# DoHoonKim8/stark-verifier

Hardware: AMD Instinct MI355X
Metric: recursive plonky2 proofs/sec (Semaphore d=20) (higher is better)
Workload: dtype u64 (Goldilocks field, integer); 1 GPU; recursive: per unit one Semaphore signal (group 2^20, n=2^13, blowup 8, 28 FRI queries, 16 PoW bits, zk) + the recursive proof verifying it (n=2^14, same FRI parameters); 128 units per GPU per step, 10 prover contexts per GPU; all_gather of (nullifier|topic) + Poseidon aggregation root per step; parallelism=independent proofs sharded over ranks, no data-path collective, exchange=none (one rank): gl355_aggregation_root over the local leaves, units_proven_in_process=1674

## Files before the change

include/gl355.h:

```cpp
#ifndef GL355_H
#define GL355_H
#include <stddef.h>
#include <stdint.h>

#ifdef __cplusplus
extern "C" {
#endif

#define GL355_OK 0
#define GL355_E_INVALID_ARG (-1)
#define GL355_E_NO_DEVICE (-2)
#define GL355_E_OOM (-3)
#define GL355_E_HIP (-4)
#define GL355_E_UNSUPPORTED (-5)
#define GL355_E_WITNESS (-6)
#define GL355_E_VERIFY (-7)

#define GL355_P UINT64_C(0xFFFFFFFF00000001)
#define GL355_COSET_SHIFT UINT64_C(7)
#define GL355_SALT_SIZE 4
#define GL355_MAX_FRI_ARITY_BITS 4
#define GL355_MAX_UNITS 16

typedef struct gl355_ctx gl355_ctx;
// ... 303 lines not shown
int32_t gl355_bn254_g1_fixed_base_mul(gl355_ctx* ctx, const uint64_t base[8], const uint64_t* scalars , uint64_t n, uint64_t* out );
int32_t gl355_bn254_g1_fft(gl355_ctx* ctx, uint64_t* points , uint32_t log_n, int32_t inverse);
typedef struct gl355_msm_bases gl355_msm_bases;
int32_t gl355_bn254_g1_msm_prepare(gl355_ctx* ctx, const uint64_t* points , uint64_t n, gl355_msm_bases** out);
int32_t gl355_bn254_g1_msm_prepared(gl355_ctx* ctx, const gl355_msm_bases* bases, const uint64_t* scalars , uint32_t n_sets,
                                    uint64_t* results );
int32_t gl355_bn254_g1_msm_bases_free(gl355_ctx* ctx, gl355_msm_bases* bases);

int32_t gl355_kzg_setup(gl355_ctx* ctx, const uint64_t tau[4], uint32_t log_n, uint64_t* g , uint64_t* g_lagrange );
int32_t gl355_kzg_lagrange_from_powers(gl355_ctx* ctx, const uint64_t* g , uint64_t n_points, uint32_t log_n,
                                       uint64_t* g_lagrange );
int32_t gl355_kzg_commit(gl355_ctx* ctx, const uint64_t* g , const uint64_t* poly , uint32_t log_n, int32_t values_form,
                         uint64_t result[8]);
int32_t gl355_kzg_open(gl355_ctx* ctx, const uint64_t* g, const uint64_t* coeffs, uint32_t log_n, const uint64_t z[4], uint64_t eval[4],
                       uint64_t witness[8], uint64_t* quotient );

typedef struct gl355_plonk_pk gl355_plonk_pk;
enum { GL355_PLONK_STAGE_ADVICE = 0, GL355_PLONK_STAGE_LOOKUP_PERMUTE = 1, GL355_PLONK_STAGE_PERMUTATION = 2, GL355_PLONK_STAGE_LOOKUP_PRODUCT = 3,
       GL355_PLONK_STAGE_VANISHING_RANDOM = 4, GL355_PLONK_STAGE_EVALUATE_H = 5, GL355_PLONK_STAGE_QUOTIENT_COMMIT = 6, GL355_PLONK_STAGE_EVALUATIONS = 7,
       GL355_PLONK_STAGE_SHPLONK = 8, GL355_PLONK_STAGES = 9 };
int32_t gl355_keccak256(const uint8_t* data, uint64_t len, uint8_t out[32]);
int32_t gl355_kzg_commit_columns(gl355_ctx* ctx, const uint64_t* g, const uint64_t* columns, uint32_t log_n, uint32_t n_cols, uint64_t* results );
int32_t gl355_plonk_keygen(gl355_ctx* ctx, const uint64_t* desc, uint64_t desc_words, const uint64_t* g, const uint64_t* g_lagrange, const uint64_t* fixed_values,
                           const uint32_t* mapping, gl355_plonk_pk** out);
int32_t gl355_plonk_pk_info(const gl355_plonk_pk* pk, uint64_t info[8]);
int32_t gl355_plonk_pk_commitments(const gl355_plonk_pk* pk, uint64_t* fixed_commitments, uint64_t* sigma_commitments);
int32_t gl355_plonk_pk_digest(const gl355_plonk_pk* pk, uint64_t digest[4]);
int32_t gl355_plonk_pk_set_digest(gl355_plonk_pk* pk, const uint64_t digest[4]);
int32_t gl355_plonk_pk_export_quotient(gl355_plonk_pk* pk, uint64_t* host_out );
int32_t gl355_plonk_prove(gl355_ctx* ctx, gl355_plonk_pk* pk, const uint64_t* advice, const uint64_t* instances, const uint32_t* instance_lens, const uint8_t seed[32],
                          uint8_t* proof, uint64_t capacity, uint64_t* proof_len, uint64_t* trace, double* stage_ms);
int32_t gl355_plonk_pk_destroy(gl355_plonk_pk* pk);

enum { GL355_PLONK_FAIL_GATE = 0, GL355_PLONK_FAIL_GATE_POISONED = 1, GL355_PLONK_FAIL_LOOKUP = 2, GL355_PLONK_FAIL_PERMUTATION = 3 };
int32_t gl355_plonk_check_witness(gl355_ctx* ctx, const uint64_t* desc, uint64_t desc_words, const uint64_t* fixed_values, const uint32_t* mapping ,
                                  const uint64_t* advice, const uint64_t* instances, const uint32_t* instance_lens, uint32_t* failures ,
                                  uint64_t capacity, uint64_t* n_failures, double* stage_ms );

typedef struct gl355_halo2_tape gl355_halo2_tape;
int32_t gl355_halo2_tape_load(gl355_ctx* ctx, const uint64_t* tape, uint64_t n_words, uint64_t n_inputs, uint32_t k, uint32_t n_advice, gl355_halo2_tape** out);
int32_t gl355_halo2_tape_free(gl355_halo2_tape* tape);
int32_t gl355_halo2_synthesize(gl355_ctx* ctx, const gl355_halo2_tape* tape, const uint64_t* inputs, uint64_t* advice_out, uint64_t* status );
int32_t gl355_halo2_tape_launches(const gl355_halo2_tape* tape, uint64_t* out );
int32_t gl355_halo2_synthesize_host(const uint64_t* tape, uint64_t n_words, uint64_t n_inputs, uint32_t k, uint32_t n_advice, const uint64_t* inputs,
                                    uint64_t* advice_out, uint64_t* status );

typedef struct gl355_plonk_vk gl355_plonk_vk;
int32_t gl355_bn254_g2_mul(const uint64_t scalar[4], const uint64_t* point , uint64_t out[16]);
int32_t gl355_bn254_pairing_check(const uint64_t* g1 , const uint64_t* g2 , uint32_t n, int32_t* ok);
int32_t gl355_plonk_vk_create(const uint64_t* desc, uint64_t desc_words, const uint64_t* fixed_commitments, const uint64_t* sigma_commitments,
                              const uint64_t digest[4] , const uint64_t s_g2[16], gl355_plonk_vk** out);
int32_t gl355_plonk_vk_from_pk(const gl355_plonk_pk* pk, const uint64_t s_g2[16], gl355_plonk_vk** out);
int32_t gl355_plonk_vk_destroy(gl355_plonk_vk* vk);
int32_t gl355_plonk_verify(gl355_ctx* ctx , const gl355_plonk_vk* vk, const uint64_t* instances, const uint32_t* instance_lens,
                           const uint8_t* proof, uint64_t proof_len, int32_t* ok);
int32_t gl355_plonk_verify_batch(gl355_ctx* ctx , const gl355_plonk_vk* vk, uint32_t n_proofs, const uint64_t* instances ,
                                 const uint32_t* instance_lens , const uint8_t* const* proofs, const uint64_t* proof_lens,
                                 const uint8_t seed[32], int32_t* ok, int32_t* first_bad );
const char* gl355_plonk_verify_last_error(void);
int32_t gl355_plonk_verify_stage_ms(double ms[3]);
int32_t gl355_kzg_params_check(gl355_ctx* ctx, const uint64_t* g , uint64_t n_points, const uint64_t* g_lagrange ,
                               uint32_t log_n, const uint64_t s_g2[16], const uint8_t seed[32], int32_t* ok);

int32_t gl355_zs_partial_products(gl355_ctx* ctx, const uint64_t* wires, const uint64_t* sigmas,
                                  const uint64_t* k_is, uint32_t log_n, uint32_t n_routed,
                                  uint32_t max_degree, uint64_t beta, uint64_t gamma,
                                  uint64_t* z_out, uint64_t* pp_out);

enum { GL355_BN_M_MUL = 0, GL355_BN_M_ADD = 1, GL355_BN_M_SUB = 2, GL355_BN_M_CANON = 3, GL355_BN_M_FROM_INT = 4, GL355_BN_M_TO_INT = 5,
       GL355_BN_M_INV = 6, GL355_BN_M_IS_ZERO = 7, GL355_BN_M_EQ = 8, GL355_BN_FQ = 16,
       GL355_BN_F29_MUL = 32, GL355_BN_F29_MUL_FR = 33, GL355_BN_F29_ADD_NORM = 34, GL355_BN_F29_SUB_C2 = 35, GL355_BN_F29_SUB_C4 = 36,
       GL355_BN_F29_SUB_C8 = 37, GL355_BN_F29_SUB_C16 = 38, GL355_BN_F29_NEG_C2 = 39, GL355_BN_F29_FROM_U256 = 40, GL355_BN_F29_TO_U256 = 41,
       GL355_BN_F29_LIFT = 42, GL355_BN_F29_LIFT_INL = 43, GL355_BN_F29_LOWER = 44, GL355_BN_F29_IS_ZERO_MOD = 45, GL355_BN_F29_TABLE_FORM = 46,
       GL355_BN_F29_NORM = 47, GL355_BN_HASH_FR_ENTER = 48, GL355_BN_HASH_FR_LEAVE = 49 };
enum { GL355_BN_CHAIN_XYZZ = 0, GL355_BN_CHAIN_JAC29 = 1, GL355_BN_CHAIN_JAC = 2, GL355_BN_CHAIN_RED29_LIFT = 3, GL355_BN_CHAIN_RED29_RAW = 4,
       GL355_BN_CHAIN_J = 5 };
enum { GL355_BN_STEP_ADD = 0, GL355_BN_STEP_DOUBLE = 1, GL355_BN_STEP_ACC = 2, GL355_BN_STEP_SELF = 3, GL355_BN_STEP_MADD = 4 };
int32_t gl355_bn254_arith_batch(gl355_ctx* ctx, int32_t op, const uint32_t* a , const uint32_t* b , uint32_t* out ,
                                uint64_t n);
int32_t gl355_bn254_g1_chain(gl355_ctx* ctx, int32_t form, const uint32_t* operands , uint32_t n_operands,
                             const uint32_t* steps , uint32_t n_chains, uint32_t n_steps, uint32_t* trace );

enum { GL355_GL_MUL = 0, GL355_GL_MUL_MULTI1 = 1, GL355_GL_MUL_MULTI2 = 2, GL355_GL_MUL_MULTI3 = 3, GL355_GL_MUL_MULTI4 = 4, GL355_GL_MUL_FILL = 5,
       GL355_GL_MUL2_FILL = 6, GL355_GL_SQR = 7, GL355_GL_SBOX = 8, GL355_GL_SBOX4 = 9, GL355_GL_RECOMBINE = 10, GL355_GL_RECOMBINE_MULTI4 = 11 };
int32_t gl355_gl_arith_batch(gl355_ctx* ctx, int32_t op, const uint64_t* a , const uint64_t* b , uint64_t* out , uint64_t n);
int32_t gl355_poseidon_permute_lanes(gl355_ctx* ctx, int32_t form, uint64_t* states , uint64_t count);


int32_t gl355_bn254_g1_msm_bits(gl355_ctx* ctx, const uint64_t* points, const gl355_msm_bases* bases , const uint64_t* scalars, uint64_t n,
                                uint32_t n_sets, uint32_t max_bits, uint64_t* results , uint32_t plan_out[4] );
int32_t gl355_plonk_pk_commit_columns(gl355_plonk_pk* pk, uint32_t which, const uint64_t* columns , uint32_t sets, uint64_t tail,
                                      uint64_t* results );

#ifdef __cplusplus
}
#endif
#endif
```

stark-verifier_amd/csrc/gl_hook.hip:

```cpp
#include "gl355_internal.h"
#include "poseidon_lanes.cuh"

namespace gl355 {

static int hk_gl_width(int32_t op) {
    switch (op) {
    case GL355_GL_MUL: case GL355_GL_MUL_MULTI1: case GL355_GL_MUL_FILL: case GL355_GL_SQR: case GL355_GL_SBOX: case GL355_GL_RECOMBINE: return 1;
    case GL355_GL_MUL_MULTI2: case GL355_GL_MUL2_FILL: return 2;
    case GL355_GL_MUL_MULTI3: return 3;
    case GL355_GL_MUL_MULTI4: case GL355_GL_SBOX4: case GL355_GL_RECOMBINE_MULTI4: return 4;
    default: return 0;
    }
}

template <int N> GL_DEV void hk_mul_multi(const uint64_t* a, const uint64_t* b, uint64_t* out) {
    uint64_t x[N], y[N], r[N];
#pragma unroll
    for (int j = 0; j < N; j++) { x[j] = a[j]; y[j] = b[j]; }
    gl_mul_multi<N>(x, y, r);
#pragma unroll
    for (int j = 0; j < N; j++) out[j] = r[j];
}

struct HkRow {
    uint64_t xr[5], al, ah;
    GL_DEV HkRow(uint64_t a, uint64_t b) {
#pragma unroll
        for (int k = 0; k < 5; k++) xr[k] = a * (uint64_t)(k + 1) + b;
        al = (uint32_t)b; ah = b >> 32;
    }
    GL_DEV void term(int k) {
        al += (uint64_t)(uint32_t)xr[k] * PSD_CIRC_DEV[k];
        ah += (uint64_t)(uint32_t)(xr[k] >> 32) * PSD_CIRC_DEV[k];
    }
};

__global__ void __launch_bounds__(256) gl_arith_hook_kernel(int32_t op, int32_t width, const uint64_t* a, const uint64_t* b, uint64_t* out, uint64_t n) {
    const uint64_t i = (blockIdx.x * (uint64_t)blockDim.x + threadIdx.x) * (uint64_t)width;
    if (i >= n) return;
    const uint64_t* pa = a + i;
    const uint64_t* pb = b + i;
    uint64_t* po = out + i;
    switch (op) {
    case GL355_GL_MUL: po[0] = gl_mul(pa[0], pb[0]); break;
    case GL355_GL_MUL_MULTI1: hk_mul_multi<1>(pa, pb, po); break;
    case GL355_GL_MUL_MULTI2: hk_mul_multi<2>(pa, pb, po); break;
    case GL355_GL_MUL_MULTI3: hk_mul_multi<3>(pa, pb, po); break;
    case GL355_GL_MUL_MULTI4: hk_mul_multi<4>(pa, pb, po); break;
    case GL355_GL_MUL_FILL: {
        HkRow row(pa[0], pb[0]);
        po[0] = gl_mul_fill(pa[0], pb[0], [&](int k) { row.term(k); });
        po[n] = row.al; po[2 * n] = row.ah;
        break;
    }
    case GL355_GL_MUL2_FILL: {
        HkRow row(pa[0], pb[0]);
        const uint64_t x[2] = {pa[0], pa[1]}, y[2] = {pb[0], pb[1]};
        uint64_t r[2];
        gl_mul2_fill(x, y, r, [&](int k) { row.term(k); });
        po[0] = r[0]; po[1] = r[1];
        po[n] = row.al; po[2 * n] = row.ah;
        po[n + 1] = 0; po[2 * n + 1] = 0;
        break;
    }
    case GL355_GL_SQR: po[0] = gl_sqr(pa[0]); break;
    case GL355_GL_SBOX: po[0] = psd_sbox(pa[0]); break;
    case GL355_GL_SBOX4: {
        uint64_t x0 = pa[0], x1 = pa[1], x2 = pa[2], x3 = pa[3];
        psd_sbox4(x0, x1, x2, x3);
        po[0] = x0; po[1] = x1; po[2] = x2; po[3] = x3;
        break;
    }
    case GL355_GL_RECOMBINE: po[0] = psd_recombine(pa[0], pb[0]); break;
    default: {
        const uint64_t al[4] = {pa[0], pa[1], pa[2], pa[3]}, ah[4] = {pb[0], pb[1], pb[2], pb[3]};
        uint64_t r[4];
        psd_recombine_multi<4>(al, ah, r);
        po[0] = r[0]; po[1] = r[1]; po[2] = r[2]; po[3] = r[3];
        break;
    }
    }
}

template <int FORM>
__global__ void __launch_bounds__(64) poseidon_lanes_hook_kernel(uint64_t* states, uint64_t count) {
    __shared__ uint64_t rings[4][24];
    const int li = threadIdx.x & 15, grp = threadIdx.x >> 4;
    uint64_t g = blockIdx.x * 4ull + grp;
    const bool valid = g < count;
    if (!valid) g = 0;
    uint64_t s = (li < 12) ? states[g * 12 + li] : 0;
    s = psd_permute_lanes<FORM>(s, li, rings[grp]);
    if (valid && li < 12) states[g * 12 + li] = gl_canon(s);
}

}

using namespace gl355;

extern "C" {
int32_t gl355_gl_arith_batch(gl355_ctx* h, int32_t op, const uint64_t* a, const uint64_t* b, uint64_t* out, uint64_t n) {
    Ctx* ctx = ctx_of(h);
    if (!ctx) return GL355_E_INVALID_ARG;
    if (hipSetDevice(ctx->device) != hipSuccess) return ctx->fail(GL355_E_HIP, "hipSetDevice failed");
    const int width = hk_gl_width(op);
    if (!width) return ctx->fail(GL355_E_INVALID_ARG, "gl_arith_batch: bad op");
    if (n % (uint64_t)width) return ctx->fail(GL355_E_INVALID_ARG, "gl_arith_batch: n is not a multiple of the op's records per lane");
    if (n == 0) return GL355_OK;
    const bool two = !(op == GL355_GL_SQR || op == GL355_GL_SBOX || op == GL355_GL_SBOX4);
    if (!a || !out || (two && !b)) return ctx->fail(GL355_E_INVALID_ARG, "gl_arith_batch: null argument");
    const uint64_t lanes = n / (uint64_t)width;
    if ((lanes + 255) / 256 > 0x7FFFFFFFull) return ctx->fail(GL355_E_UNSUPPORTED, "gl_arith_batch: too many records");
    const uint64_t out_words = (op == GL355_GL_MUL_FILL || op == GL355_GL_MUL2_FILL) ? 3 * n : n;
    Staged sa(ctx), sb(ctx), so(ctx);
    GL355_TRY(sa.open(a, n * 8, 1));
    GL355_TRY(sb.open(two ? b : a, n * 8, 1));
    GL355_TRY(so.open(out, out_words * 8, 2));
    hipLaunchKernelGGL(gl_arith_hook_kernel, dim3((uint32_t)((lanes + 255) / 256)), dim3(256), 0, ctx->stream, op, (int32_t)width, sa.as<const uint64_t>(),
                       sb.as<const uint64_t>(), so.as<uint64_t>(), n);
    GL355_HIP(ctx, hipGetLastError());
    return so.finish();
}

int32_t gl355_poseidon_permute_lanes(gl355_ctx* h, int32_t form, uint64_t* states, uint64_t count) {
    Ctx* ctx = ctx_of(h);
    if (!ctx) return GL355_E_INVALID_ARG;
    if (hipSetDevice(ctx->device) != hipSuccess) return ctx->fail(GL355_E_HIP, "hipSetDevice failed");
    if (form != 0 && form != 3) return ctx->fail(GL355_E_INVALID_ARG, "poseidon_permute_lanes: form is 0 or 3");
    if (count == 0) return GL355_OK;
    if (!states) return ctx->fail(GL355_E_INVALID_ARG, "poseidon_permute_lanes: null states");
    if ((count + 3) / 4 > 0x7FFFFFFFull) return ctx->fail(GL355_E_UNSUPPORTED, "poseidon_permute_lanes: too many states");
    Staged s(ctx);
    GL355_TRY(s.open(states, count * 96, 3));
    const dim3 grid((uint32_t)((count + 3) / 4)), block(64);
    if (form == 3) hipLaunchKernelGGL(poseidon_lanes_hook_kernel<3>, grid, block, 0, ctx->stream, s.as<uint64_t>(), count);
    else hipLaunchKernelGGL(poseidon_lanes_hook_kernel<0>, grid, block, 0, ctx->stream, s.as<uint64_t>(), count);
    GL355_HIP(ctx, hipGetLastError());
    return s.finish();
}
}
```

stark-verifier_amd/csrc/poseidon.cuh:

```cuda
#pragma once
#include "gl_field.cuh"
#if GL_MUL_VARIANT != 1
#error "poseidon.cuh is written on the inline-asm product and its lock-step groups: GL_MUL_VARIANT 1"
#endif

#define PSD_TABLE_QUAL __device__ __constant__ const
#include "poseidon_tables.h"

namespace gl355 {

GL_DEV uint64_t psd_sbox(uint64_t x) {
    const uint64_t x2 = gl_sqr(x);
    const uint64_t a[2] = {x, x2}, b[2] = {x2, x2};
    uint64_t r[2];
    gl_mul_multi<2>(a, b, r);
    return gl_mul(r[0], r[1]);
}

GL_DEV uint64_t psd_recombine(uint64_t al, uint64_t ah) {
    uint32_t t1 = (uint32_t)(al >> 32), top;
    asm("v_add_co_u32_e32 %0, vcc, %0, %2\n\t" GL_HAZARD_NOP "v_addc_co_u32_e32 %1, vcc, 0, %3, vcc"
        : "+v"(t1), "=v"(top) : "v"((uint32_t)ah), "v"((uint32_t)(ah >> 32)) : "vcc");
    return gl_dev_add_mul_eps(((uint64_t)t1 << 32) | (uint32_t)al, top);
}

GL_DEV void psd_sbox4(uint64_t& x0, uint64_t& x1, uint64_t& x2, uint64_t& x3) {
    const uint64_t a[4] = {x0, x1, x2, x3};
    uint64_t sq[4], c3[4], c4[4], o[4];
    gl_mul_multi<4>(a, a, sq);
    gl_mul_multi<4>(a, sq, c3);
    gl_mul_multi<4>(sq, sq, c4);
    gl_mul_multi<4>(c3, c4, o);
    x0 = o[0]; x1 = o[1]; x2 = o[2]; x3 = o[3];
}
template <int N>
GL_DEV void psd_recombine_multi(const uint64_t (&al)[N], const uint64_t (&ah)[N], uint64_t (&out)[N]) {
    static_assert(N >= 3, "three or more: no wait states of their own");
    uint32_t t1[N], top[N], m[N];
    uint64_t c[N], r[N];
#pragma unroll
    for (int j = 0; j < N; j++) {
        asm("v_add_co_u32_e64 %0, %1, %2, %3" : "=v"(t1[j]), "=s"(c[j]) : "v"((uint32_t)(al[j] >> 32)), "v"((uint32_t)ah[j]));
        __builtin_amdgcn_sched_barrier(0);
    }
#pragma unroll
    for (int j = 0; j < N; j++) {
        asm("v_addc_co_u32_e64 %0, %1, 0, %2, %1" : "=v"(top[j]), "+s"(c[j]) : "v"((uint32_t)(ah[j] >> 32)));
        __builtin_amdgcn_sched_barrier(0);
    }
#pragma unroll
    for (int j = 0; j < N; j++) {
        const uint64_t x = ((uint64_t)t1[j] << 32) | (uint32_t)al[j];
        asm("v_mad_u64_u32 %0, %1, %2, -1, %3" : "=v"(r[j]), "=s"(c[j]) : "v"(top[j]), "v"(x));
        __builtin_amdgcn_sched_barrier(0);
    }
#pragma unroll
    for (int j = 0; j < N; j++) {
        asm("v_cndmask_b32_e64 %0, 0, -1, %1" : "=v"(m[j]) : "s"(c[j]));
        __builtin_amdgcn_sched_barrier(0);
    }
#pragma unroll
    for (int j = 0; j < N; j++) out[j] = r[j] + (uint64_t)m[j];
}

#define PSD_MDS_CHAIN(C0)                                                                                  \
    "v_mad_u64_u32 %0, %1, %2, " #C0 ", %14\n\tv_mad_u64_u32 %0, %1, %3, 15, %0\n\tv_mad_u64_u32 %0, %1, %4, 41, %0\n\t" \
    "v_mad_u64_u32 %0, %1, %5, 16, %0\n\tv_mad_u64_u32 %0, %1, %6, 2, %0\n\tv_mad_u64_u32 %0, %1, %7, 28, %0\n\t"      \
    "v_mad_u64_u32 %0, %1, %8, 13, %0\n\tv_mad_u64_u32 %0, %1, %9, 13, %0\n\tv_mad_u64_u32 %0, %1, %10, 39, %0\n\t"    \
    "v_mad_u64_u32 %0, %1, %11, 18, %0\n\tv_mad_u64_u32 %0, %1, %12, 34, %0\n\tv_mad_u64_u32 %0, %1, %13, 20, %0"
template <int R>
GL_DEV uint64_t psd_mds_chain(const uint32_t (&x)[12], uint64_t addend) {
    uint64_t acc, unused;
#define PSD_X(i) "v"(x[((i) + R) % 12])
    if constexpr (R == 0)
        asm(PSD_MDS_CHAIN(25) : "=&v"(acc), "=&s"(unused) : PSD_X(0), PSD_X(1), PSD_X(2), PSD_X(3), PSD_X(4), PSD_X(5), PSD_X(6),
            PSD_X(7), PSD_X(8), PSD_X(9), PSD_X(10), PSD_X(11), "s"(addend));
    else
        asm(PSD_MDS_CHAIN(17) : "=&v"(acc), "=&s"(unused) : PSD_X(0), PSD_X(1), PSD_X(2), PSD_X(3), PSD_X(4), PSD_X(5), PSD_X(6),
            PSD_X(7), PSD_X(8), PSD_X(9), PSD_X(10), PSD_X(11), "s"(addend));
#undef PSD_X
    return acc;
}
template <int R>
GL_DEV void psd_mds_rows(uint64_t (&s)[12], const uint32_t (&lo)[12], const uint32_t (&hi)[12], const uint64_t* rc) {
    if constexpr (R < 12) {
        const uint64_t c0 = rc[R], c1 = rc[R + 1], c2 = rc[R + 2], c3 = rc[R + 3];
        const uint64_t al[4] = {psd_mds_chain<R>(lo, (uint32_t)c0), psd_mds_chain<R + 1>(lo, (uint32_t)c1), psd_mds_chain<R + 2>(lo, (uint32_t)c2),
                                psd_mds_chain<R + 3>(lo, (uint32_t)c3)};
        const uint64_t ah[4] = {psd_mds_chain<R>(hi, c0 >> 32), psd_mds_chain<R + 1>(hi, c1 >> 32), psd_mds_chain<R + 2>(hi, c2 >> 32),
                                psd_mds_chain<R + 3>(hi, c3 >> 32)};
        uint64_t o[4];
        __builtin_amdgcn_sched_barrier(0);
        psd_recombine_multi<4>(al, ah, o);
        s[R] = o[0]; s[R + 1] = o[1]; s[R + 2] = o[2]; s[R + 3] = o[3];
        psd_mds_rows<R + 4>(s, lo, hi, rc);
    }
}
GL_DEV void psd_mds(uint64_t (&s)[12], const uint64_t* rc) {
    uint32_t lo[12], hi[12];
#pragma unroll
    for (int i = 0; i < 12; i++) { lo[i] = (uint32_t)s[i]; hi[i] = (uint32_t)(s[i] >> 32); }
    psd_mds_rows<0>(s, lo, hi, rc);
}


#undef PSD_TABLE_QUAL
#define PSD_TABLE_QUAL __device__ __constant__
#include "poseidon_ktables.h"

GL_DEV void psd_split(uint64_t x, uint32_t (&l)[3]) {
    const uint32_t lo = (uint32_t)x, hi = (uint32_t)(x >> 32);
    l[0] = lo & 0x3FFFFFu;
    l[1] = __builtin_amdgcn_alignbit(hi, lo, 22) & 0x3FFFFFu;
    l[2] = hi >> 12;
}
typedef const __attribute__((address_space(4))) uint64_t* psd_ktab;
GL_DEV void psd_mac(uint64_t& lo, uint64_t& hi, const uint32_t (&l)[3], const uint64_t (&c)[3]) {
    const uint64_t c0 = c[0], c1 = c[1], c2 = c[2];
    uint64_t unused;
    asm("v_mad_u64_u32 %0, %2, %3, %9, %0\n\tv_mad_u64_u32 %1, %2, %4, %9, %1\n\t"
        "v_mad_u64_u32 %0, %2, %5, %10, %0\n\tv_mad_u64_u32 %1, %2, %6, %10, %1\n\t"
        "v_mad_u64_u32 %0, %2, %7, %11, %0\n\tv_mad_u64_u32 %1, %2, %8, %11, %1"
        : "+v"(lo), "+v"(hi), "=&s"(unused)
        : "s"((uint32_t)c0), "s"((uint32_t)(c0 >> 32)), "s"((uint32_t)c1), "s"((uint32_t)(c1 >> 32)), "s"((uint32_t)c2), "s"((uint32_t)(c2 >> 32)),
          "v"(l[0]), "v"(l[1]), "v"(l[2]));
}
GL_DEV void psd_mac_first(uint64_t& lo, uint64_t& hi, const uint32_t (&l)[3], const uint64_t (&c)[3], const uint64_t (&add)[2]) {
    const uint64_t c0 = c[0], c1 = c[1], c2 = c[2];
    uint64_t unused;
    asm("v_mov_b64 %0, %12\n\tv_mov_b64 %1, %13\n\t"
        "v_mad_u64_u32 %0, %2, %3, %9, %0\n\tv_mad_u64_u32 %1, %2, %4, %9, %1\n\t"
        "v_mad_u64_u32 %0, %2, %5, %10, %0\n\tv_mad_u64_u32 %1, %2, %6, %10, %1\n\t"
        "v_mad_u64_u32 %0, %2, %7, %11, %0\n\tv_mad_u64_u32 %1, %2, %8, %11, %1"
        : "=&v"(lo), "=&v"(hi), "=&s"(unused)
        : "s"((uint32_t)c0), "s"((uint32_t)(c0 >> 32)), "s"((uint32_t)c1), "s"((uint32_t)(c1 >> 32)), "s"((uint32_t)c2), "s"((uint32_t)(c2 >> 32)),
          "v"(l[0]), "v"(l[1]), "v"(l[2]), "s"(add[0]), "s"(add[1]));
}
constexpr int psd_k_group = 5;
struct PsdK {
    uint64_t w[psd_k_group][3];
    uint64_t a[2];
};
template <int N, bool WITH_ADD>
GL_DEV void psd_kload(PsdK& k, psd_ktab c, psd_ktab add) {
#pragma unroll
    for (int i = 0; i < N; i++)
#pragma unroll
        for (int j = 0; j < 3; j++) k.w[i][j] = c[3 * i + j];
    if constexpr (WITH_ADD) { k.a[0] = add[0]; k.a[1] = add[1]; }
}
template <int NX, bool HAS_NEXT, int XCAP>
GL_DEV void psd_dot(const uint32_t (&ul)[11][3], const uint32_t (&xl)[XCAP][3], psd_ktab c, PsdK& k, psd_ktab add_next, uint64_t& lo, uint64_t& hi) {
    constexpr int G = psd_k_group, NT = 11 + NX, NG = (NT + G - 1) / G;
    PsdK cur = k;
#pragma unroll
    for (int g = 0; g < NG; g++) {
        const int n = NT - g * G < G ? NT - g * G : G;
        PsdK nxt;
#pragma unroll
        for (int i = 0; i < G; i++) {
            const int t = g * G + i;
            if (t == 0) psd_mac_first(lo, hi, ul[0], cur.w[0], cur.a);
            else if (i < n) {
                if (t < 11) psd_mac(lo, hi, ul[t], cur.w[i]);
                else psd_mac(lo, hi, xl[t - 11], cur.w[i]);
            }
            if (i == 0) {
                __builtin_amdgcn_sched_barrier(0);
                if (g + 1 < NG) {
                    if (NT - (g + 1) * G >= G) psd_kload<G, false>(nxt, c + 3 * (g + 1) * G, add_next);
                    else psd_kload<(NT % G ? NT % G : G), false>(nxt, c + 3 * (g + 1) * G, add_next);
                } else if constexpr (HAS_NEXT) {
                    psd_kload<G, true>(nxt, c + 3 * NT, add_next);
                }
                __builtin_amdgcn_sched_barrier(0);
            }
        }
        __builtin_amdgcn_sched_barrier(0);
        if (g + 1 < NG || HAS_NEXT) cur = nxt;
    }
    if constexpr (HAS_NEXT) k = cur;
}
template <int J>
GL_DEV void psd_block_lane0(const uint32_t (&ul)[11][3], uint32_t (&xl)[PSD_K_BLOCK][3], psd_ktab mac, psd_ktab add, PsdK& k) {
    if constexpr (J < PSD_K_BLOCK) {
        uint64_t lo, hi;
        psd_dot<J, true>(ul, xl, mac + 3 * (11 * (J - 1) + (J - 1) * J / 2), k, add + 2 * J, lo, hi);
        psd_split(psd_sbox(psd_recombine(lo, hi)), xl[J]);
        __builtin_amdgcn_sched_barrier(0);
        psd_block_lane0<J + 1>(ul, xl, mac, add, k);
    }
}
template <int R>
GL_DEV void psd_block_out(uint64_t (&s)[12], const uint32_t (&ul)[11][3], const uint32_t (&xl)[PSD_K_BLOCK][3], psd_ktab mac, psd_ktab add, PsdK& k) {
    constexpr int B = PSD_K_BLOCK;
    if constexpr (R < 12) {
        uint64_t lo, hi;
        psd_dot<B, (R < 11)>(ul, xl, mac + 3 * (11 * (B - 1) + (B - 1) * B / 2 + (11 + B) * R), k, add + 2 * (B + R), lo, hi);
        s[R] = psd_recombine(lo, hi);
        __builtin_amdgcn_sched_barrier(0);
        psd_block_out<R + 1>(s, ul, xl, mac, add, k);
    }
}
GL_DEV void psd_partial_rounds_block(uint64_t (&s)[12]) {
    constexpr int B = PSD_K_BLOCK;
#pragma unroll 1
    for (int blk = 0; blk < 22 / B; blk++) {
        psd_ktab add = (psd_ktab)PSD_K_ADD + blk * 2 * (B - 1 + 12);
        psd_ktab mac = (psd_ktab)PSD_K_MAC;
        asm volatile("" : "+s"(mac));
        PsdK k;
        psd_kload<psd_k_group, true>(k, mac, add);
        __builtin_amdgcn_sched_barrier(0);
        uint32_t ul[11][3], xl[B][3];
#pragma unroll
        for (int i = 0; i < 11; i++) psd_split(s[i + 1], ul[i]);
        psd_split(psd_sbox(s[0]), xl[0]);
        __builtin_amdgcn_sched_barrier(0);
        psd_block_lane0<1>(ul, xl, mac, add, k);
        psd_block_out<0>(s, ul, xl, mac, add, k);
    }
}

constexpr int psd_rounds_per_iter = 2;
GL_DEV void psd_dense_rounds(uint64_t (&s)[12], int r0, int r1) {
#pragma unroll 1
    for (int r = r0; r < r1; r += psd_rounds_per_iter) {
#pragma unroll
        for (int h = 0; h < psd_rounds_per_iter; h++) {
#pragma unroll
            for (int i = 0; i < 12; i += 4) psd_sbox4(s[i], s[i + 1], s[i + 2], s[i + 3]);
            psd_mds(s, &PSD_ALL_RC[12 * (r + h + 1)]);
        }
    }
}
GL_DEV void psd_permute(uint64_t (&s)[12]) {
#pragma unroll
    for (int i = 0; i < 12; i++) s[i] = gl_add_canonical(s[i], PSD_ALL_RC[i]);
    psd_dense_rounds(s, 0, 4);
    psd_partial_rounds_block(s);
    psd_dense_rounds(s, 26, 30);
}

struct PsdSponge {
    uint64_t s[12];
    GL_DEV void init() {
#pragma unroll
        for (int i = 0; i < 12; i++) s[i] = 0;
    }
};

}
```

Baseline: 332.1 recursive proofs/s.

## Restructure Poseidon partial rounds into 3-round blocks with small MDS-derived constants

Replaces the old partial-round block scheme, which split state limbs into 22-bit pieces and used 64-bit constants, with a new 3-round block form. Each output is now a dot product of full 32-bit halves times small (22-bit or narrower) constants, using two mad_u64_u32 per term. This runs 7 blocks of 3 rounds (21) plus one final sbox and MDS round, with new precomputed tables. It also adds a test hook op for the partial rounds. The intent is to cut multiply count and scalar-constant loads in the Poseidon hot path. The risk lies in accumulator overflow bounds and the correctness of the new tables.

```diff
diff --git a/include/gl355.h b/include/gl355.h
--- a/include/gl355.h
+++ b/include/gl355.h
@@ -409,7 +409,8 @@
                              const uint32_t* steps , uint32_t n_chains, uint32_t n_steps, uint32_t* trace );
 
 enum { GL355_GL_MUL = 0, GL355_GL_MUL_MULTI1 = 1, GL355_GL_MUL_MULTI2 = 2, GL355_GL_MUL_MULTI3 = 3, GL355_GL_MUL_MULTI4 = 4, GL355_GL_MUL_FILL = 5,
-       GL355_GL_MUL2_FILL = 6, GL355_GL_SQR = 7, GL355_GL_SBOX = 8, GL355_GL_SBOX4 = 9, GL355_GL_RECOMBINE = 10, GL355_GL_RECOMBINE_MULTI4 = 11 };
+       GL355_GL_MUL2_FILL = 6, GL355_GL_SQR = 7, GL355_GL_SBOX = 8, GL355_GL_SBOX4 = 9, GL355_GL_RECOMBINE = 10, GL355_GL_RECOMBINE_MULTI4 = 11,
+       GL355_GL_PARTIAL_ROUNDS = 13 };
 int32_t gl355_gl_arith_batch(gl355_ctx* ctx, int32_t op, const uint64_t* a , const uint64_t* b , uint64_t* out , uint64_t n);
 int32_t gl355_poseidon_permute_lanes(gl355_ctx* ctx, int32_t form, uint64_t* states , uint64_t count);
 
diff --git a/stark-verifier_amd/csrc/gl_hook.hip b/stark-verifier_amd/csrc/gl_hook.hip
--- a/stark-verifier_amd/csrc/gl_hook.hip
+++ b/stark-verifier_amd/csrc/gl_hook.hip
@@ -9,6 +9,7 @@
     case GL355_GL_MUL_MULTI2: case GL355_GL_MUL2_FILL: return 2;
     case GL355_GL_MUL_MULTI3: return 3;
     case GL355_GL_MUL_MULTI4: case GL355_GL_SBOX4: case GL355_GL_RECOMBINE_MULTI4: return 4;
+    case GL355_GL_PARTIAL_ROUNDS: return 12;
     default: return 0;
     }
 }
@@ -72,6 +73,15 @@
         break;
     }
     case GL355_GL_RECOMBINE: po[0] = psd_recombine(pa[0], pb[0]); break;
+    case GL355_GL_PARTIAL_ROUNDS: {
+        uint64_t s[12];
+#pragma unroll
+        for (int j = 0; j < 12; j++) s[j] = pa[j];
+        psd_partial_rounds_b3(s);
+#pragma unroll
+        for (int j = 0; j < 12; j++) po[j] = s[j];
+        break;
+    }
     default: {
         const uint64_t al[4] = {pa[0], pa[1], pa[2], pa[3]}, ah[4] = {pb[0], pb[1], pb[2], pb[3]};
         uint64_t r[4];
@@ -107,7 +117,7 @@
     if (!width) return ctx->fail(GL355_E_INVALID_ARG, "gl_arith_batch: bad op");
     if (n % (uint64_t)width) return ctx->fail(GL355_E_INVALID_ARG, "gl_arith_batch: n is not a multiple of the op's records per lane");
     if (n == 0) return GL355_OK;
-    const bool two = !(op == GL355_GL_SQR || op == GL355_GL_SBOX || op == GL355_GL_SBOX4);
+    const bool two = !(op == GL355_GL_SQR || op == GL355_GL_SBOX || op == GL355_GL_SBOX4 || op == GL355_GL_PARTIAL_ROUNDS);
     if (!a || !out || (two && !b)) return ctx->fail(GL355_E_INVALID_ARG, "gl_arith_batch: null argument");
     const uint64_t lanes = n / (uint64_t)width;
     if ((lanes + 255) / 256 > 0x7FFFFFFFull) return ctx->fail(GL355_E_UNSUPPORTED, "gl_arith_batch: too many records");
diff --git a/stark-verifier_amd/csrc/poseidon.cuh b/stark-verifier_amd/csrc/poseidon.cuh
--- a/stark-verifier_amd/csrc/poseidon.cuh
+++ b/stark-verifier_amd/csrc/poseidon.cuh
@@ -81,8 +81,8 @@
 #undef PSD_X
     return acc;
 }
-template <int R>
-GL_DEV void psd_mds_rows(uint64_t (&s)[12], const uint32_t (&lo)[12], const uint32_t (&hi)[12], const uint64_t* rc) {
+template <int R, class RC>
+GL_DEV void psd_mds_rows(uint64_t (&s)[12], const uint32_t (&lo)[12], const uint32_t (&hi)[12], RC rc) {
     if constexpr (R < 12) {
         const uint64_t c0 = rc[R], c1 = rc[R + 1], c2 = rc[R + 2], c3 = rc[R + 3];
         const uint64_t al[4] = {psd_mds_chain<R>(lo, (uint32_t)c0), psd_mds_chain<R + 1>(lo, (uint32_t)c1), psd_mds_chain<R + 2>(lo, (uint32_t)c2),
@@ -93,133 +93,112 @@
         __builtin_amdgcn_sched_barrier(0);
         psd_recombine_multi<4>(al, ah, o);
         s[R] = o[0]; s[R + 1] = o[1]; s[R + 2] = o[2]; s[R + 3] = o[3];
-        psd_mds_rows<R + 4>(s, lo, hi, rc);
-    }
-}
-GL_DEV void psd_mds(uint64_t (&s)[12], const uint64_t* rc) {
+        psd_mds_rows<R + 4, RC>(s, lo, hi, rc);
+    }
+}
+template <class RC>
+GL_DEV void psd_mds(uint64_t (&s)[12], RC rc) {
     uint32_t lo[12], hi[12];
 #pragma unroll
     for (int i = 0; i < 12; i++) { lo[i] = (uint32_t)s[i]; hi[i] = (uint32_t)(s[i] >> 32); }
-    psd_mds_rows<0>(s, lo, hi, rc);
+    psd_mds_rows<0, RC>(s, lo, hi, rc);
 }
 
 
 #undef PSD_TABLE_QUAL
 #define PSD_TABLE_QUAL __device__ __constant__
-#include "poseidon_ktables.h"
-
-GL_DEV void psd_split(uint64_t x, uint32_t (&l)[3]) {
-    const uint32_t lo = (uint32_t)x, hi = (uint32_t)(x >> 32);
-    l[0] = lo & 0x3FFFFFu;
-    l[1] = __builtin_amdgcn_alignbit(hi, lo, 22) & 0x3FFFFFu;
-    l[2] = hi >> 12;
-}
-typedef const __attribute__((address_space(4))) uint64_t* psd_ktab;
-GL_DEV void psd_mac(uint64_t& lo, uint64_t& hi, const uint32_t (&l)[3], const uint64_t (&c)[3]) {
-    const uint64_t c0 = c[0], c1 = c[1], c2 = c[2];
+#include "poseidon_b3tables.h"
+
+typedef const __attribute__((address_space(4))) uint32_t* psd_b3tab;
+typedef const __attribute__((address_space(4))) uint64_t* psd_b3add;
+GL_DEV void psd_b3_term(uint64_t& lo, uint64_t& hi, uint32_t c, uint64_t v) {
     uint64_t unused;
-    asm("v_mad_u64_u32 %0, %2, %3, %9, %0\n\tv_mad_u64_u32 %1, %2, %4, %9, %1\n\t"
-        "v_mad_u64_u32 %0, %2, %5, %10, %0\n\tv_mad_u64_u32 %1, %2, %6, %10, %1\n\t"
-        "v_mad_u64_u32 %0, %2, %7, %11, %0\n\tv_mad_u64_u32 %1, %2, %8, %11, %1"
+    asm("v_mad_u64_u32 %0, %2, %3, %4, %0\n\tv_mad_u64_u32 %1, %2, %3, %5, %1"
+        : "+v"(lo), "+v"(hi), "=&s"(unused) : "s"(c), "v"((uint32_t)v), "v"((uint32_t)(v >> 32)));
+}
+GL_DEV void psd_b3_terms5(uint64_t& lo, uint64_t& hi, const uint32_t* c, const uint64_t* v) {
+    uint64_t unused;
+#define PSD_V(i) "v"((uint32_t)v[i]), "v"((uint32_t)(v[i] >> 32))
+    asm("v_mad_u64_u32 %0, %2, %3, %8, %0\n\tv_mad_u64_u32 %1, %2, %3, %9, %1\n\t"
+        "v_mad_u64_u32 %0, %2, %4, %10, %0\n\tv_mad_u64_u32 %1, %2, %4, %11, %1\n\t"
+        "v_mad_u64_u32 %0, %2, %5, %12, %0\n\tv_mad_u64_u32 %1, %2, %5, %13, %1\n\t"
+        "v_mad_u64_u32 %0, %2, %6, %14, %0\n\tv_mad_u64_u32 %1, %2, %6, %15, %1\n\t"
+        "v_mad_u64_u32 %0, %2, %7, %16, %0\n\tv_mad_u64_u32 %1, %2, %7, %17, %1"
         : "+v"(lo), "+v"(hi), "=&s"(unused)
-        : "s"((uint32_t)c0), "s"((uint32_t)(c0 >> 32)), "s"((uint32_t)c1), "s"((uint32_t)(c1 >> 32)), "s"((uint32_t)c2), "s"((uint32_t)(c2 >> 32)),
-          "v"(l[0]), "v"(l[1]), "v"(l[2]));
-}
-GL_DEV void psd_mac_first(uint64_t& lo, uint64_t& hi, const uint32_t (&l)[3], const uint64_t (&c)[3], const uint64_t (&add)[2]) {
-    const uint64_t c0 = c[0], c1 = c[1], c2 = c[2];
+        : "s"(c[0]), "s"(c[1]), "s"(c[2]), "s"(c[3]), "s"(c[4]), PSD_V(0), PSD_V(1), PSD_V(2), PSD_V(3), PSD_V(4));
+#undef PSD_V
+}
+GL_DEV void psd_b3_term_first(uint64_t& lo, uint64_t& hi, uint32_t c, uint64_t v, const uint64_t (&add)[2]) {
     uint64_t unused;
-    asm("v_mov_b64 %0, %12\n\tv_mov_b64 %1, %13\n\t"
-        "v_mad_u64_u32 %0, %2, %3, %9, %0\n\tv_mad_u64_u32 %1, %2, %4, %9, %1\n\t"
-        "v_mad_u64_u32 %0, %2, %5, %10, %0\n\tv_mad_u64_u32 %1, %2, %6, %10, %1\n\t"
-        "v_mad_u64_u32 %0, %2, %7, %11, %0\n\tv_mad_u64_u32 %1, %2, %8, %11, %1"
-        : "=&v"(lo), "=&v"(hi), "=&s"(unused)
-        : "s"((uint32_t)c0), "s"((uint32_t)(c0 >> 32)), "s"((uint32_t)c1), "s"((uint32_t)(c1 >> 32)), "s"((uint32_t)c2), "s"((uint32_t)(c2 >> 32)),
-          "v"(l[0]), "v"(l[1]), "v"(l[2]), "s"(add[0]), "s"(add[1]));
-}
-constexpr int psd_k_group = 5;
-struct PsdK {
-    uint64_t w[psd_k_group][3];
+    asm("v_mov_b64 %0, %6\n\tv_mov_b64 %1, %7\n\t"
+        "v_mad_u64_u32 %0, %2, %3, %4, %0\n\tv_mad_u64_u32 %1, %2, %3, %5, %1"
+        : "=&v"(lo), "=&v"(hi), "=&s"(unused) : "s"(c), "v"((uint32_t)v), "v"((uint32_t)(v >> 32)), "s"(add[0]), "s"(add[1]));
+}
+struct PsdB3Row {
+    uint32_t w[14];
     uint64_t a[2];
 };
-template <int N, bool WITH_ADD>
-GL_DEV void psd_kload(PsdK& k, psd_ktab c, psd_ktab add) {
-#pragma unroll
-    for (int i = 0; i < N; i++)
-#pragma unroll
-        for (int j = 0; j < 3; j++) k.w[i][j] = c[3 * i + j];
-    if constexpr (WITH_ADD) { k.a[0] = add[0]; k.a[1] = add[1]; }
-}
-template <int NX, bool HAS_NEXT, int XCAP>
-GL_DEV void psd_dot(const uint32_t (&ul)[11][3], const uint32_t (&xl)[XCAP][3], psd_ktab c, PsdK& k, psd_ktab add_next, uint64_t& lo, uint64_t& hi) {
-    constexpr int G = psd_k_group, NT = 11 + NX, NG = (NT + G - 1) / G;
-    PsdK cur = k;
-#pragma unroll
-    for (int g = 0; g < NG; g++) {
-        const int n = NT - g * G < G ? NT - g * G : G;
-        PsdK nxt;
-#pragma unroll
-        for (int i = 0; i < G; i++) {
-            const int t = g * G + i;
-            if (t == 0) psd_mac_first(lo, hi, ul[0], cur.w[0], cur.a);
-            else if (i < n) {
-                if (t < 11) psd_mac(lo, hi, ul[t], cur.w[i]);
-                else psd_mac(lo, hi, xl[t - 11], cur.w[i]);
-            }
-            if (i == 0) {
-                __builtin_amdgcn_sched_barrier(0);
-                if (g + 1 < NG) {
-                    if (NT - (g + 1) * G >= G) psd_kload<G, false>(nxt, c + 3 * (g + 1) * G, add_next);
-                    else psd_kload<(NT % G ? NT % G : G), false>(nxt, c + 3 * (g + 1) * G, add_next);
-                } else if constexpr (HAS_NEXT) {
-                    psd_kload<G, true>(nxt, c + 3 * NT, add_next);
-                }
-                __builtin_amdgcn_sched_barrier(0);
-            }
-        }
-        __builtin_amdgcn_sched_barrier(0);
-        if (g + 1 < NG || HAS_NEXT) cur = nxt;
-    }
-    if constexpr (HAS_NEXT) k = cur;
-}
-template <int J>
-GL_DEV void psd_block_lane0(const uint32_t (&ul)[11][3], uint32_t (&xl)[PSD_K_BLOCK][3], psd_ktab mac, psd_ktab add, PsdK& k) {
-    if constexpr (J < PSD_K_BLOCK) {
-        uint64_t lo, hi;
-        psd_dot<J, true>(ul, xl, mac + 3 * (11 * (J - 1) + (J - 1) * J / 2), k, add + 2 * J, lo, hi);
-        psd_split(psd_sbox(psd_recombine(lo, hi)), xl[J]);
-        __builtin_amdgcn_sched_barrier(0);
-        psd_block_lane0<J + 1>(ul, xl, mac, add, k);
-    }
+template <int NT>
+GL_DEV void psd_b3_load(PsdB3Row& k, psd_b3tab c, psd_b3add add) {
+#pragma unroll
+    for (int i = 0; i < NT; i++) k.w[i] = c[i];
+    k.a[0] = add[0]; k.a[1] = add[1];
+}
+template <int NX, int NT_NEXT>
+GL_DEV void psd_b3_dot(const uint64_t (&u)[12], const uint64_t (&x)[3], PsdB3Row& k, psd_b3tab next, psd_b3add add_next, uint64_t& lo, uint64_t& hi) {
+    const PsdB3Row cur = k;
+    psd_b3_term_first(lo, hi, cur.w[0], u[1], cur.a);
+    __builtin_amdgcn_sched_barrier(0);
+    if constexpr (NT_NEXT > 0) psd_b3_load<NT_NEXT>(k, next, add_next);
+    __builtin_amdgcn_sched_barrier(0);
+    psd_b3_terms5(lo, hi, &cur.w[1], &u[2]);
+    psd_b3_terms5(lo, hi, &cur.w[6], &u[7]);
+#pragma unroll
+    for (int t = 0; t < NX; t++) psd_b3_term(lo, hi, cur.w[11 + t], x[t]);
+    __builtin_amdgcn_sched_barrier(0);
 }
 template <int R>
-GL_DEV void psd_block_out(uint64_t (&s)[12], const uint32_t (&ul)[11][3], const uint32_t (&xl)[PSD_K_BLOCK][3], psd_ktab mac, psd_ktab add, PsdK& k) {
-    constexpr int B = PSD_K_BLOCK;
+GL_DEV void psd_b3_out(uint64_t (&o)[12], const uint64_t (&u)[12], const uint64_t (&x)[3], psd_b3tab mac, psd_b3add add, PsdB3Row& k) {
     if constexpr (R < 12) {
-        uint64_t lo, hi;
-        psd_dot<B, (R < 11)>(ul, xl, mac + 3 * (11 * (B - 1) + (B - 1) * B / 2 + (11 + B) * R), k, add + 2 * (B + R), lo, hi);
-        s[R] = psd_recombine(lo, hi);
-        __builtin_amdgcn_sched_barrier(0);
-        psd_block_out<R + 1>(s, ul, xl, mac, add, k);
-    }
-}
-GL_DEV void psd_partial_rounds_block(uint64_t (&s)[12]) {
-    constexpr int B = PSD_K_BLOCK;
+        constexpr int W = PSD_B3_ROW_WORDS;
+        uint64_t al[4], ah[4], r[4];
+        psd_b3_dot<3, 14>(u, x, k, mac + W * (R + 3), add + 2 * (R + 3), al[0], ah[0]);
+        psd_b3_dot<3, 14>(u, x, k, mac + W * (R + 4), add + 2 * (R + 4), al[1], ah[1]);
+        psd_b3_dot<3, 14>(u, x, k, mac + W * (R + 5), add + 2 * (R + 5), al[2], ah[2]);
+        psd_b3_dot<3, (R + 3 < 11 ? 14 : 0)>(u, x, k, mac + W * (R + 6), add + 2 * (R + 6), al[3], ah[3]);
+        psd_recombine_multi<4>(al, ah, r);
+        o[R] = r[0]; o[R + 1] = r[1]; o[R + 2] = r[2]; o[R + 3] = r[3];
+        __builtin_amdgcn_sched_barrier(0);
+        psd_b3_out<R + 4>(o, u, x, mac, add, k);
+    }
+}
+GL_DEV void psd_partial_rounds_b3(uint64_t (&s)[12]) {
 #pragma unroll 1
-    for (int blk = 0; blk < 22 / B; blk++) {
-        psd_ktab add = (psd_ktab)PSD_K_ADD + blk * 2 * (B - 1 + 12);
-        psd_ktab mac = (psd_ktab)PSD_K_MAC;
-        asm volatile("" : "+s"(mac));
-        PsdK k;
-        psd_kload<psd_k_group, true>(k, mac, add);
-        __builtin_amdgcn_sched_barrier(0);
-        uint32_t ul[11][3], xl[B][3];
-#pragma unroll
-        for (int i = 0; i < 11; i++) psd_split(s[i + 1], ul[i]);
-        psd_split(psd_sbox(s[0]), xl[0]);
-        __builtin_amdgcn_sched_barrier(0);
-        psd_block_lane0<1>(ul, xl, mac, add, k);
-        psd_block_out<0>(s, ul, xl, mac, add, k);
-    }
+    for (int blk = 0; blk < PSD_B3_BLOCKS; blk++) {
+        constexpr int W = PSD_B3_ROW_WORDS;
+        psd_b3add add = (psd_b3add)PSD_B3_ADD + blk * 2 * 14;
+        psd_b3tab mac = (psd_b3tab)PSD_B3_MAC;
+        asm volatile("" : "+s"(mac), "+s"(add));
+        PsdB3Row k;
+        psd_b3_load<12>(k, mac, add);
+        __builtin_amdgcn_sched_barrier(0);
+        uint64_t x[3], o[12], lo, hi;
+        x[0] = psd_sbox(s[0]);
+        __builtin_amdgcn_sched_barrier(0);
+        psd_b3_dot<1, 13>(s, x, k, mac + W, add + 2, lo, hi);
+        x[1] = psd_sbox(psd_recombine(lo, hi));
+        __builtin_amdgcn_sched_barrier(0);
+        psd_b3_dot<2, 14>(s, x, k, mac + 2 * W, add + 4, lo, hi);
+        x[2] = psd_sbox(psd_recombine(lo, hi));
+        __builtin_amdgcn_sched_barrier(0);
+        psd_b3_out<0>(o, s, x, mac, add, k);
+#pragma unroll
+        for (int i = 0; i < 12; i++) s[i] = o[i];
+    }
+    psd_b3add rc26 = (psd_b3add)PSD_ALL_RC + 12 * 26;
+    asm volatile("" : "+s"(rc26));
+    s[0] = psd_sbox(s[0]);
+    psd_mds(s, rc26);
 }
 
 constexpr int psd_rounds_per_iter = 2;
@@ -238,7 +217,7 @@
 #pragma unroll
     for (int i = 0; i < 12; i++) s[i] = gl_add_canonical(s[i], PSD_ALL_RC[i]);
     psd_dense_rounds(s, 0, 4);
-    psd_partial_rounds_block(s);
+    psd_partial_rounds_b3(s);
     psd_dense_rounds(s, 26, 30);
 }
 
diff --git a/stark-verifier_amd/csrc/poseidon_b3tables.h b/stark-verifier_amd/csrc/poseidon_b3tables.h
--- /dev/null
+++ b/stark-verifier_amd/csrc/poseidon_b3tables.h
@@ -0,0 +1,74 @@
+#pragma once
+#include <stdint.h>
+#ifndef PSD_TABLE_QUAL
+#define PSD_TABLE_QUAL static const
+#endif
+#define PSD_B3_BLOCKS 7
+#define PSD_B3_ROW_WORDS 16
+PSD_TABLE_QUAL uint32_t PSD_B3_MAC[224] = {
+  0x00000fu, 0x000029u, 0x000010u, 0x000002u, 0x00001cu, 0x00000du, 0x00000du, 0x000027u, 0x000012u, 0x000022u, 0x000014u, 0x000019u, 0x000000u, 0x000000u, 0x000000u, 0x000000u,
+  0x0015c9u, 0x000f31u, 0x001368u, 0x00182cu, 0x001230u, 0x001371u, 0x00167bu, 0x00131fu, 0x00114eu, 0x001750u, 0x001300u, 0x001399u, 0x000019u, 0x000000u, 0x000000u, 0x000000u,
+  0x128961u, 0x10a091u, 0x134fc0u, 0x132c94u, 0x117c58u, 0x13f8a1u, 0x124d03u, 0x10cf7fu, 0x134a96u, 0x10b6c8u, 0x11f718u, 0x1336c9u, 0x001399u, 0x000019u, 0x000000u, 0x000000u,
+  0x12ffacu, 0x10c158u, 0x122b3cu, 0x13d930u, 0x114c04u, 0x1268c8u, 0x1386b4u, 0x104168u, 0x1274e4u, 0x116070u, 0x11f13cu, 0x11f718u, 0x001300u, 0x000014u, 0x000000u, 0x000000u,
+  0x107460u, 0x0fc768u, 0x1105b0u, 0x118ba0u, 0x10aef0u, 0x110f88u, 0x10ad20u, 0x0fe138u, 0x10c000u, 0x0ebee0u, 0x116070u, 0x10b6c8u, 0x001750u, 0x000022u, 0x000000u, 0x000000u,
+  0x12662au, 0x10d0aeu, 0x135efcu, 0x135a88u, 0x11a73cu, 0x1396d6u, 0x126bceu, 0x10cc32u, 0x13cc18u, 0x10c000u, 0x1274e4u, 0x134a96u, 0x00114eu, 0x000012u, 0x000000u, 0x000000u,
+  0x114e8fu, 0x0f392fu, 0x108868u, 0x120a2cu, 0x100d68u, 0x10e427u, 0x115e4du, 0x0eb881u, 0x10cc32u, 0x0fe138u, 0x104168u, 0x10cf7fu, 0x00131fu, 0x000027u, 0x000000u, 0x000000u,
+  0x12c387u, 0x116343u, 0x129204u, 0x136fb4u, 0x126a3cu, 0x13066bu, 0x12a0e5u, 0x115e4du, 0x126bceu, 0x10ad20u, 0x1386b4u, 0x124d03u, 0x00167bu, 0x00000du, 0x000000u, 0x000000u,
+  0x128cd9u, 0x1136e9u, 0x13a4b0u, 0x13a0f4u, 0x11b3a8u, 0x13df99u, 0x13066bu, 0x10e427u, 0x1396d6u, 0x110f88u, 0x1268c8u, 0x13f8a1u, 0x001371u, 0x00000du, 0x000000u, 0x000000u,
+  0x12c1e4u, 0x0ff958u, 0x11dcc4u, 0x1318f0u, 0x10d53cu, 0x11b3a8u, 0x126a3cu, 0x100d68u, 0x11a73cu, 0x10aef0u, 0x114c04u, 0x117c58u, 0x001230u, 0x00001cu, 0x000000u, 0x000000u,
+  0x135dbcu, 0x124db4u, 0x132cf0u, 0x14dbf0u, 0x1318f0u, 0x13a0f4u, 0x136fb4u, 0x120a2cu, 0x135a88u, 0x118ba0u, 0x13d930u, 0x132c94u, 0x00182cu, 0x000002u, 0x000000u, 0x000000u,
+  0x12615cu, 0x10bb98u, 0x13d294u, 0x132cf0u, 0x11dcc4u, 0x13a4b0u, 0x129204u, 0x108868u, 0x135efcu, 0x1105b0u, 0x122b3cu, 0x134fc0u, 0x001368u, 0x000010u, 0x000000u, 0x000000u,
+  0x115b61u, 0x0fa3a1u, 0x10bb98u, 0x124db4u, 0x0ff958u, 0x1136e9u, 0x116343u, 0x0f392fu, 0x10d0aeu, 0x0fc768u, 0x10c158u, 0x10a091u, 0x000f31u, 0x000029u, 0x000000u, 0x000000u,
+  0x12581du, 0x115b61u, 0x12615cu, 0x135dbcu, 0x12c1e4u, 0x128cd9u, 0x12c387u, 0x114e8fu, 0x12662au, 0x107460u, 0x12ffacu, 0x128961u, 0x0015c9u, 0x00000fu, 0x000000u, 0x000000u,
+};
+PSD_TABLE_QUAL uint64_t PSD_B3_ADD[196] = {
+  UINT64_C(0x00000000268d7d8c), UINT64_C(0x000000007131aa45), UINT64_C(0x00000000de0778d0), UINT64_C(0x00000000f1417c86),
+  UINT64_C(0x000000001ef1f717), UINT64_C(0x00000000be56ca78), UINT64_C(0x00000000a029077b), UINT64_C(0x000000009a8644b3),
+  UINT64_C(0x00000000268817e7), UINT64_C(0x0000000052b02192), UINT64_C(0x00000000582f33a3), UINT64_C(0x000000000abc5297),
+  UINT64_C(0x000000007990679a), UINT64_C(0x00000000e54f22ee), UINT64_C(0x00000000a2518f18), UINT64_C(0x00000000a469d6ae),
+  UINT64_C(0x0000000037b273cc), UINT64_C(0x00000000bb1b667d), UINT64_C(0x00000000a2a4519d), UINT64_C(0x000000003c358ffb),
+  UINT64_C(0x00000000410f63fa), UINT64_C(0x00000000be01b370), UINT64_C(0x000000008b5714f8), UINT64_C(0x00000000d5ba62f7),
+  UINT64_C(0x00000000d89243c8), UINT64_C(0x0000000020bf71b9), UINT64_C(0x0000000070c921f3), UINT64_C(0x000000007af4c52b),
+  UINT64_C(0x00000000c3ac118e), UINT64_C(0x000000007159cd30), UINT64_C(0x000000006ff4f0e2), UINT64_C(0x000000003efc7580),
+  UINT64_C(0x00000000fd0a553b), UINT64_C(0x00000000854e26e7), UINT64_C(0x00000000a714d050), UINT64_C(0x000000006e2d494d),
+  UINT64_C(0x00000000b9653dfd), UINT64_C(0x0000000015536d53), UINT64_C(0x000000003f2ac720), UINT64_C(0x00000000dc1b3579),
+  UINT64_C(0x00000000d71b5368), UINT64_C(0x00000000371b585e), UINT64_C(0x000000003e2320ab), UINT64_C(0x000000004ca149f2),
+  UINT64_C(0x000000000194e8f8), UINT64_C(0x000000007c4fd5da), UINT64_C(0x00000000a5ac26e0), UINT64_C(0x0000000044d6d6ea),
+  UINT64_C(0x00000000e6151b8f), UINT64_C(0x000000006e4712cf), UINT64_C(0x00000000e0558d8a), UINT64_C(0x0000000044680366),
+  UINT64_C(0x000000006da2cab4), UINT64_C(0x000000000839ba7c), UINT64_C(0x00000000e2327e99), UINT64_C(0x00000000586a9fb8),
+  UINT64_C(0x0000000093258387), UINT64_C(0x0000000030a46805), UINT64_C(0x000000009b604341), UINT64_C(0x00000000c750352d),
+  UINT64_C(0x0000000066e3abc2), UINT64_C(0x00000000d6b93cc9), UINT64_C(0x0000000052289282), UINT64_C(0x0000000036ee51b4),
+  UINT64_C(0x00000000458f7d4d), UINT64_C(0x000000001bb20c3a), UINT64_C(0x00000000ac80cdfa), UINT64_C(0x000000001ffdfb49),
+  UINT64_C(0x00000000298022d5), UINT64_C(0x000000000fa800e4), UINT64_C(0x00000000b996bbc1), UINT64_C(0x00000000dbf976a1),
+  UINT64_C(0x0000000076f2d4d5), UINT64_C(0x00000000225b39a1), UINT64_C(0x0000000069082198), UINT64_C(0x00000000a45d5e6b),
+  UINT64_C(0x00000000fa675720), UINT64_C(0x000000003809a401), UINT64_C(0x00000000b5c50370), UINT64_C(0x00000000c2e6704c),
+  UINT64_C(0x0000000065fbbcd7), UINT64_C(0x000000001d5e6b28), UINT64_C(0x000000004bb5e49f), UINT64_C(0x0000000046333421),
+  UINT64_C(0x000000002d74d7f7), UINT64_C(0x0000000077500598), UINT64_C(0x000000008a73b798), UINT64_C(0x000000003fe3eee0),
+  UINT64_C(0x00000000d77d2177), UINT64_C(0x0000000066809a1b), UINT64_C(0x000000006b7b1a7b), UINT64_C(0x0000000025bd84ce),
+  UINT64_C(0x000000003047b692), UINT64_C(0x00000000de59fdea), UINT64_C(0x0000000010178af1), UINT64_C(0x0000000075fb00dd),
+  UINT64_C(0x000000002d9c33ce), UINT64_C(0x0000000046556f5c), UINT64_C(0x00000000bd25de10), UINT64_C(0x00000000699471c4),
+  UINT64_C(0x00000000632059cb), UINT64_C(0x000000002a6ebf09), UINT64_C(0x000000008b8c3be9), UINT64_C(0x00000000a17b5803),
+  UINT64_C(0x0000000082537744), UINT64_C(0x000000008fc747be), UINT64_C(0x00000000429da700), UINT64_C(0x00000000790d302d),
+  UINT64_C(0x00000000fdf0055e), UINT64_C(0x000000002c41991a), UINT64_C(0x00000000c6bfc0ab), UINT64_C(0x0000000032f3edef),
+  UINT64_C(0x0000000000c17442), UINT64_C(0x00000000dd611f10), UINT64_C(0x00000000fac93576), UINT64_C(0x00000000e44c4dd5),
+  UINT64_C(0x00000000d41b033f), UINT64_C(0x0000000015f154a2), UINT64_C(0x0000000029688609), UINT64_C(0x00000000d1795c6e),
+  UINT64_C(0x00000000116c6ec1), UINT64_C(0x00000000f3267319), UINT64_C(0x00000000ad93b9cc), UINT64_C(0x0000000074ee383c),
+  UINT64_C(0x00000000fcd44819), UINT64_C(0x00000000ca17dcb4), UINT64_C(0x0000000036869a7e), UINT64_C(0x0000000028eb017c),
+  UINT64_C(0x00000000c49a303d), UINT64_C(0x00000000d8c39810), UINT64_C(0x00000000f4f8d367), UINT64_C(0x0000000091a5e951),
+  UINT64_C(0x000000008c856749), UINT64_C(0x00000000b14f64de), UINT64_C(0x00000000c32305f1), UINT64_C(0x000000000e0f4582),
+  UINT64_C(0x0000000086f7685a), UINT64_C(0x000000005def8c2e), UINT64_C(0x00000000c28f9600), UINT64_C(0x00000000166054a2),
+  UINT64_C(0x00000000d5d01d33), UINT64_C(0x00000000e89cd854), UINT64_C(0x00000000988250a0), UINT64_C(0x0000000044e8d81a),
+  UINT64_C(0x0000000053a3e603), UINT64_C(0x000000006fa19061), UINT64_C(0x0000000014b1b0f2), UINT64_C(0x000000002f293617),
+  UINT64_C(0x0000000086303ee1), UINT64_C(0x00000000fcb08855), UINT64_C(0x00000000e4dde9b3), UINT64_C(0x000000002e17c5d7),
+  UINT64_C(0x0000000053fe1c65), UINT64_C(0x0000000058d33908), UINT64_C(0x0000000047d8dced), UINT64_C(0x00000000aebfdda0),
+  UINT64_C(0x00000000e5747ec6), UINT64_C(0x00000000675d6c7a), UINT64_C(0x00000000d25def23), UINT64_C(0x0000000027732879),
+  UINT64_C(0x000000005ccc86e5), UINT64_C(0x00000000b8d35c9d), UINT64_C(0x00000000081bafe9), UINT64_C(0x000000004fe2afbe),
+  UINT64_C(0x00000000d78e7686), UINT64_C(0x00000000fd1e3e36), UINT64_C(0x00000000f66def9c), UINT64_C(0x00000000b18169e4),
+  UINT64_C(0x00000000e9a39368), UINT64_C(0x00000000de122beb), UINT64_C(0x000000005d2e95d9), UINT64_C(0x00000000a7529fb8),
+  UINT64_C(0x000000007870a682), UINT64_C(0x00000000ab5eb4de), UINT64_C(0x00000000fa73f523), UINT64_C(0x000000006ae79d56),
+  UINT64_C(0x00000000357ef8a2), UINT64_C(0x00000000f650f4f4), UINT64_C(0x0000000018f720d6), UINT64_C(0x00000000a140ca88),
+  UINT64_C(0x00000000fe62eb20), UINT64_C(0x00000000bc531094), UINT64_C(0x0000000019911c1d), UINT64_C(0x00000000b2b726df),
+  UINT64_C(0x00000000c761c075), UINT64_C(0x0000000077c73890), UINT64_C(0x00000000cc7702db), UINT64_C(0x000000005d605fb1),
+  UINT64_C(0x0000000026a636be), UINT64_C(0x000000002965bb99), UINT64_C(0x000000007855c471), UINT64_C(0x00000000530cc006),
+  UINT64_C(0x00000000c93c9b30), UINT64_C(0x00000000abc50207), UINT64_C(0x00000000eb195297), UINT64_C(0x00000000063f5cc2),
+};
```

Measured after the change: 363.6 recursive proofs/s, median of 6. 1.09x the previous value.
